# neu-vi/Superpoints_Registration

Measured on AMD Instinct MI355X. Metric: point-cloud pairs/sec (16 384 pts/cloud), higher is better.
Workload: dtype f32 (matrix products: range-scaled split-f16x2 MFMA, f32 accumulate; attention weights below 2^-5 of their row sum carried in one f16 plane); 1 GPU; synthetic 16384-pt pairs, full KPConv backbone + superpoint attn + Sinkhorn-SVD pose (3dmatch config, BASELINE configs[1]); streams_per_gpu=1, points_per_cloud=16384, generator=box, point_order=reference, upsample_indices=True, cross_step_overlap=True, streams_inside_a_forward=3: main path, pyramid searches, ResNet shortcut branches

## Files before the change

superpoints_registration_amd/csrc/norm_pool.hip:

```cpp
#include "spr_common.h"

namespace spr {
namespace {

constexpr int kSliceRows = 512;
int in_nsplit(int max_len) {
  int s = cdiv(max_len > 0 ? max_len : 1, kSliceRows);
  return s < 1 ? 1 : s;
}

__global__ __launch_bounds__(256) void k_in_stats(const float* __restrict__ x,
                                                  const int* __restrict__ cu, int c, int nsplit,
                                                  double* __restrict__ part ) {
  const int cloud = blockIdx.x, split = blockIdx.y, cb = blockIdx.z * 64;
  const int beg = cu[cloud], end = cu[cloud + 1];
  const int r0 = beg + split * kSliceRows;
  const int r1 = min(r0 + kSliceRows, end);
  const int cw = min(c - cb, 64);
  const int cw4 = cw >> 2;
  const int rl = 256 / cw4;
  const int tc = threadIdx.x % cw4, tr = threadIdx.x / cw4;
  __shared__ double sh[8][256];
  double s[4] = {0, 0, 0, 0}, ss[4] = {0, 0, 0, 0};
  if (tr < rl) {
    const float* base = x + cb + 4 * tc;
    int r = r0 + tr;
    for (; r + 3 * rl < r1; r += 4 * rl) {
      float4 v[4];
#pragma unroll
      for (int u = 0; u < 4; ++u)
        v[u] = *reinterpret_cast<const float4*>(base + (size_t)(r + u * rl) * c);
#pragma unroll
      for (int u = 0; u < 4; ++u) {
        const double a = v[u].x, b = v[u].y, cc = v[u].z, d = v[u].w;
        s[0] += a; ss[0] += a * a;
        s[1] += b; ss[1] += b * b;
        s[2] += cc; ss[2] += cc * cc;
        s[3] += d; ss[3] += d * d;
      }
    }
    for (; r < r1; r += rl) {
      const float4 v = *reinterpret_cast<const float4*>(base + (size_t)r * c);
      const double a = v.x, b = v.y, cc = v.z, d = v.w;
      s[0] += a; ss[0] += a * a;
      s[1] += b; ss[1] += b * b;
      s[2] += cc; ss[2] += cc * cc;
      s[3] += d; ss[3] += d * d;
    }
  }
#pragma unroll
  for (int k = 0; k < 4; ++k) {
    sh[k][threadIdx.x] = s[k];
    sh[4 + k][threadIdx.x] = ss[k];
  }
  __syncthreads();
  if (tr == 0) {
    double* p = part + (((size_t)cloud * nsplit + split) * 2) * c;
#pragma unroll
    for (int k = 0; k < 4; ++k) {
      double a = s[k], b = ss[k];
      for (int q = 1; q < rl; ++q) {
        a += sh[k][q * cw4 + tc];
        b += sh[4 + k][q * cw4 + tc];
      }
      p[cb + 4 * tc + k] = a;
      p[c + cb + 4 * tc + k] = b;
    }
  }
}

__global__ void k_in_final(const double* __restrict__ part, const int* __restrict__ cu, int nb,
                           int c, int nsplit, float eps, float* __restrict__ mean,
                           float* __restrict__ rstd) {
  const int i = blockIdx.x * blockDim.x + threadIdx.x;
  if (i >= nb * c) return;
  const int cloud = i / c, ch = i % c;
  double s = 0.0, ss = 0.0;
  for (int k = 0; k < nsplit; ++k) {
    const double* p = part + (((size_t)cloud * nsplit + k) * 2) * c;
    s += p[ch];
    ss += p[c + ch];
  }
  const int len = cu[cloud + 1] - cu[cloud];
  const double n = len > 0 ? (double)len : 1.0;
  const double m = s / n;
  double var = ss / n - m * m;
  if (var < 0.0) var = 0.0;
  mean[i] = (float)m;
  rstd[i] = (float)(1.0 / sqrt(var + (double)eps));
}

__device__ __forceinline__ void publish_range(float mx, float* __restrict__ slots, int nslots) {
  __shared__ float shr[4];
  mx = wave_max(mx);
  if ((threadIdx.x & 63) == 0) shr[threadIdx.x >> 6] = mx;
  __syncthreads();
  if (threadIdx.x == 0)
    atomicMax(reinterpret_cast<unsigned int*>(slots) + (blockIdx.x & (nslots - 1)),
              __float_as_uint(fmaxf(fmaxf(shr[0], shr[1]), fmaxf(shr[2], shr[3]))));
}

constexpr int kInApplyUnroll = 4;
__global__ __launch_bounds__(256) void k_in_apply(const float* __restrict__ x, const int* __restrict__ cu, int n,
                                                  int nb, int c, int norm, const float* __restrict__ mean,
                                                  const float* __restrict__ rstd, const float* __restrict__ add,
                                                  float slope, float* __restrict__ out,
                                                  float* __restrict__ out_range, int nslots) {
  const int c4 = c >> 2;
  const long total = (long)n * c4;
  const long stride = (long)gridDim.x * blockDim.x;
  const long g0 = (long)blockIdx.x * blockDim.x + threadIdx.x;
  float4 v[kInApplyUnroll], a[kInApplyUnroll];
#pragma unroll
  for (int u = 0; u < kInApplyUnroll; ++u) {
    const long gid = g0 + u * stride;
    if (gid < total) {
      v[u] = reinterpret_cast<const float4*>(x)[gid];
      if (add) a[u] = reinterpret_cast<const float4*>(add)[gid];
    }
  }
  float mx = 0.f;
#pragma unroll
  for (int u = 0; u < kInApplyUnroll; ++u) {
    const long gid = g0 + u * stride;
    if (gid >= total) continue;
    float4 w = v[u];
    if (norm) {
      const int row = (int)(gid / c4), q = (int)(gid % c4);
      const int cloud = find_segment(cu, nb, row);
      const float4 m = reinterpret_cast<const float4*>(mean + (size_t)cloud * c)[q];
      const float4 r = reinterpret_cast<const float4*>(rstd + (size_t)cloud * c)[q];
      w.x = (w.x - m.x) * r.x;
      w.y = (w.y - m.y) * r.y;
      w.z = (w.z - m.z) * r.z;
      w.w = (w.w - m.w) * r.w;
    }
    if (add) {
      w.x += a[u].x;
      w.y += a[u].y;
      w.z += a[u].z;
      w.w += a[u].w;
    }
    w.x = w.x >= 0.f ? w.x : w.x * slope;
    w.y = w.y >= 0.f ? w.y : w.y * slope;
    w.z = w.z >= 0.f ? w.z : w.z * slope;
    w.w = w.w >= 0.f ? w.w : w.w * slope;
    reinterpret_cast<float4*>(out)[gid] = w;
    mx = fmaxf(mx, fmaxf(fmaxf(fabsf(w.x), fabsf(w.y)), fmaxf(fabsf(w.z), fabsf(w.w))));
  }
  if (out_range != nullptr) publish_range(mx, out_range, nslots);
}

__global__ __launch_bounds__(256) void k_in_bwd_stats(const float* __restrict__ x, const float* __restrict__ out,
                                                      const float* __restrict__ dout, const int* __restrict__ cu,
                                                      int c, int nsplit, float slope,
                                                      const float* __restrict__ mean, const float* __restrict__ rstd,
                                                      double* __restrict__ part ) {
  const int cloud = blockIdx.x, split = blockIdx.y, cb = blockIdx.z * 64;
  const int beg = cu[cloud], end = cu[cloud + 1];
  const int r0 = beg + split * kSliceRows;
  const int r1 = min(r0 + kSliceRows, end);
  const int cw = min(c - cb, 64);
  const int cw4 = cw >> 2;
  const int rl = 256 / cw4;
  const int tc = threadIdx.x % cw4, tr = threadIdx.x / cw4;
  __shared__ double sh[8][256];
  double s1[4] = {0, 0, 0, 0}, s2[4] = {0, 0, 0, 0};
  if (tr < rl) {
    const int col = cb + 4 * tc;
    const float4 mu = *reinterpret_cast<const float4*>(mean + (size_t)cloud * c + col);
    const float4 rs = *reinterpret_cast<const float4*>(rstd + (size_t)cloud * c + col);
    for (int r = r0 + tr; r < r1; r += rl) {
      const size_t o = (size_t)r * c + col;
      const float4 xv = *reinterpret_cast<const float4*>(x + o);
      const float4 ov = *reinterpret_cast<const float4*>(out + o);
      const float4 dv = *reinterpret_cast<const float4*>(dout + o);
      const float g0 = dv.x * (ov.x > 0.f ? 1.f : slope), g1 = dv.y * (ov.y > 0.f ? 1.f : slope);
      const float g2 = dv.z * (ov.z > 0.f ? 1.f : slope), g3 = dv.w * (ov.w > 0.f ? 1.f : slope);
      s1[0] += (double)g0; s2[0] += (double)g0 * (double)((xv.x - mu.x) * rs.x);
      s1[1] += (double)g1; s2[1] += (double)g1 * (double)((xv.y - mu.y) * rs.y);
      s1[2] += (double)g2; s2[2] += (double)g2 * (double)((xv.z - mu.z) * rs.z);
      s1[3] += (double)g3; s2[3] += (double)g3 * (double)((xv.w - mu.w) * rs.w);
    }
  }
#pragma unroll
  for (int k = 0; k < 4; ++k) {
    sh[k][threadIdx.x] = s1[k];
    sh[4 + k][threadIdx.x] = s2[k];
  }
  __syncthreads();
  if (tr == 0) {
    double* p = part + (((size_t)cloud * nsplit + split) * 2) * c;
#pragma unroll
    for (int k = 0; k < 4; ++k) {
      double a = s1[k], b = s2[k];
      for (int q = 1; q < rl; ++q) {
        a += sh[k][q * cw4 + tc];
        b += sh[4 + k][q * cw4 + tc];
      }
      p[cb + 4 * tc + k] = a;
      p[c + cb + 4 * tc + k] = b;
    }
  }
}

__global__ void k_in_bwd_final(const double* __restrict__ part, const int* __restrict__ cu, int nb, int c,
                               int nsplit, double* __restrict__ m1, double* __restrict__ m2) {
  const int i = blockIdx.x * blockDim.x + threadIdx.x;
  if (i >= nb * c) return;
  const int cloud = i / c, ch = i % c;
  double s1 = 0.0, s2 = 0.0;
  for (int k = 0; k < nsplit; ++k) {
    const double* p = part + (((size_t)cloud * nsplit + k) * 2) * c;
    s1 += p[ch];
    s2 += p[c + ch];
  }
  const int len = cu[cloud + 1] - cu[cloud];
  const double n = len > 0 ? (double)len : 1.0;
  m1[i] = s1 / n;
  m2[i] = s2 / n;
}

__global__ void k_in_bwd_apply(const float* __restrict__ x, const float* __restrict__ out,
                               const float* __restrict__ dout, const int* __restrict__ cu, int n, int nb, int c,
                               int norm, float slope, const float* __restrict__ mean,
                               const float* __restrict__ rstd, const double* __restrict__ m1,
                               const double* __restrict__ m2, float* __restrict__ dx, float* __restrict__ dadd) {
  const long gid = (long)blockIdx.x * blockDim.x + threadIdx.x;
  if (gid >= (long)n * c) return;
  const int row = (int)(gid / c), ch = (int)(gid % c);
  const float g = dout[gid] * (out[gid] > 0.f ? 1.f : slope);
  if (dadd) dadd[gid] = g;
  if (!norm) {
    dx[gid] = g;
    return;
  }
  const int cloud = find_segment(cu, nb, row);
  const size_t s = (size_t)cloud * c + ch;
  const float xh = (x[gid] - mean[s]) * rstd[s];
  dx[gid] = rstd[s] * (float)(((double)g - m1[s]) - (double)xh * m2[s]);
}

__global__ void k_in_bwd_apply4(const float* __restrict__ x, const float* __restrict__ out,
                                const float* __restrict__ dout, const int* __restrict__ cu, int n, int nb, int c,
                                int norm, float slope, const float* __restrict__ mean,
                                const float* __restrict__ rstd, const double* __restrict__ m1,
                                const double* __restrict__ m2, float* __restrict__ dx, float* __restrict__ dadd) {
  const int c4 = c >> 2;
  const long gid = (long)blockIdx.x * blockDim.x + threadIdx.x;
  if (gid >= (long)n * c4) return;
  const int row = (int)(gid / c4), ch = 4 * (int)(gid % c4);
  const float4 d4 = reinterpret_cast<const float4*>(dout)[gid], o4 = reinterpret_cast<const float4*>(out)[gid];
  float g[4] = {d4.x * (o4.x > 0.f ? 1.f : slope), d4.y * (o4.y > 0.f ? 1.f : slope),
                d4.z * (o4.z > 0.f ? 1.f : slope), d4.w * (o4.w > 0.f ? 1.f : slope)};
  if (dadd) reinterpret_cast<float4*>(dadd)[gid] = make_float4(g[0], g[1], g[2], g[3]);
  if (!norm) {
    reinterpret_cast<float4*>(dx)[gid] = make_float4(g[0], g[1], g[2], g[3]);
    return;
  }
  const int cloud = find_segment(cu, nb, row);
  const size_t s = (size_t)cloud * c + ch;
  const float4 x4 = reinterpret_cast<const float4*>(x)[gid];
  const float xv[4] = {x4.x, x4.y, x4.z, x4.w};
  float r[4];
#pragma unroll
  for (int e = 0; e < 4; ++e) {
    const float xh = (xv[e] - mean[s + e]) * rstd[s + e];
    r[e] = rstd[s + e] * (float)(((double)g[e] - m1[s + e]) - (double)xh * m2[s + e]);
  }
  reinterpret_cast<float4*>(dx)[gid] = make_float4(r[0], r[1], r[2], r[3]);
}

__global__ void k_maxpool(const float* __restrict__ x, int ns, int c, const int* __restrict__ idx,
                          int nq, int idx_stride, int k, float* __restrict__ out, float* __restrict__ out_range,
                          int nslots, const int* __restrict__ order) {
  const int c4 = c >> 2;
  long gid = (long)blockIdx.x * blockDim.x + threadIdx.x;
  if (order != nullptr) gid = ((long)(blockIdx.x & 7) * (gridDim.x >> 3) + (blockIdx.x >> 3)) * blockDim.x + threadIdx.x;
  float mx = 0.f;
  if (gid < (long)nq * c4) {
  const int q = (int)(gid % c4);
  const int row = order != nullptr ? order[gid / c4] : (int)(gid / c4);
  gid = (long)row * c4 + q;
  float4 m = make_float4(-INFINITY, -INFINITY, -INFINITY, -INFINITY);
  const int* ir = idx + (size_t)row * idx_stride;
  int j = 0;
  for (; j + 4 <= k; j += 4) {
    int id[4];
    float4 v[4];
#pragma unroll
    for (int u = 0; u < 4; ++u) id[u] = ir[j + u];
#pragma unroll
    for (int u = 0; u < 4; ++u) {
      v[u] = make_float4(0.f, 0.f, 0.f, 0.f);
      if (id[u] >= 0 && id[u] < ns) v[u] = reinterpret_cast<const float4*>(x + (size_t)id[u] * c)[q];
    }
#pragma unroll
    for (int u = 0; u < 4; ++u) {
      m.x = fmaxf(m.x, v[u].x);
      m.y = fmaxf(m.y, v[u].y);
      m.z = fmaxf(m.z, v[u].z);
      m.w = fmaxf(m.w, v[u].w);
    }
  }
  for (; j < k; ++j) {
    const int id = ir[j];
    float4 v = make_float4(0.f, 0.f, 0.f, 0.f);
    if (id >= 0 && id < ns) v = reinterpret_cast<const float4*>(x + (size_t)id * c)[q];
    m.x = fmaxf(m.x, v.x);
    m.y = fmaxf(m.y, v.y);
    m.z = fmaxf(m.z, v.z);
    m.w = fmaxf(m.w, v.w);
  }
  reinterpret_cast<float4*>(out)[gid] = m;
  mx = fmaxf(fmaxf(fabsf(m.x), fabsf(m.y)), fmaxf(fabsf(m.z), fabsf(m.w)));
  }
  if (out_range != nullptr) publish_range(mx, out_range, nslots);
}

__global__ void k_gather_rows(const float* __restrict__ x, int n_src, int c,
                              const int* __restrict__ idx, int n, float* __restrict__ out) {
  const long gid = (long)blockIdx.x * blockDim.x + threadIdx.x;
  if (gid >= (long)n * c) return;
  const int row = (int)(gid / c), ch = (int)(gid % c);
  const int id = idx[row];
  out[gid] = (id >= 0 && id < n_src) ? x[(size_t)id * c + ch] : 0.f;
}

}
}

using namespace spr;

extern "C" size_t spr_instnorm_workspace_bytes(int max_len, int nb, int c) {
  const size_t B = (size_t)(nb > 0 ? nb : 1), C = (size_t)(c > 0 ? c : 1);
  const int ns = in_nsplit(max_len);
  return align_up(B * ns * 2 * C * sizeof(double), 256) + 2 * align_up(B * C * sizeof(float), 256);
}

extern "C" int spr_instnorm(const float* x, const int* cu, int n, int nb, int max_len_host, int c,
                            float eps, int norm, const float* add, float slope, float* out, float* out_range,
                            int out_range_n, void* ws, size_t ws_bytes, void* stream_) {
  hipStream_t stream = (hipStream_t)stream_;
  SPR_REQUIRE(out_range == nullptr || (out_range_n >= 1 && (out_range_n & (out_range_n - 1)) == 0),
              "instnorm: out_range_n must be a power of two");
  SPR_REQUIRE(n > 0 && nb >= 1 && c >= 4 && c % 4 == 0, "instnorm: need n>0 and c %% 4 == 0 (c=%d)", c);
  float* mean = nullptr;
  float* rstd = nullptr;
  if (norm) {
    SPR_REQUIRE(max_len_host >= 1 && max_len_host <= n, "instnorm: bad max_len_host=%d", max_len_host);
    SPR_REQUIRE(ws_bytes >= spr_instnorm_workspace_bytes(max_len_host, nb, c), "instnorm: workspace too small");
    Workspace w(ws, ws_bytes);
    const int nsplit = in_nsplit(max_len_host);
    double* part = w.take<double>((size_t)nb * nsplit * 2 * c);
    mean = w.take<float>((size_t)nb * c);
    rstd = w.take<float>((size_t)nb * c);
    SPR_REQUIRE(rstd != nullptr, "instnorm: workspace carve failed");
    hipLaunchKernelGGL(k_in_stats, dim3(nb, nsplit, cdiv(c, 64)), dim3(256), 0, stream, x, cu, c, nsplit, part);
    hipLaunchKernelGGL(k_in_final, dim3(cdiv((long)nb * c, 256)), dim3(256), 0, stream, part, cu,
                       nb, c, nsplit, eps, mean, rstd);
    SPR_LAUNCH_CHECK();
  }
  const long total = (long)n * (c / 4);
  hipLaunchKernelGGL(k_in_apply, dim3(cdiv(total, 256 * kInApplyUnroll)), dim3(256), 0, stream, x, cu, n, nb, c,
                     norm, mean, rstd, add, slope, out, out_range, out_range_n);
  SPR_LAUNCH_CHECK();
  return 0;
}

extern "C" int spr_instnorm_stats(const float* x, const int* cu, int n, int nb, int max_len_host, int c, float eps,
                                  float* mean, float* rstd, void* ws, size_t ws_bytes, void* stream_) {
  hipStream_t stream = (hipStream_t)stream_;
  SPR_REQUIRE(x && cu && mean && rstd && n > 0 && nb >= 1 && c >= 4 && c % 4 == 0, "instnorm_stats: bad arguments (c=%d)", c);
  SPR_REQUIRE(max_len_host >= 1 && max_len_host <= n, "instnorm_stats: bad max_len_host=%d", max_len_host);
  SPR_REQUIRE(ws_bytes >= spr_instnorm_workspace_bytes(max_len_host, nb, c), "instnorm_stats: workspace too small");
  Workspace w(ws, ws_bytes);
  const int nsplit = in_nsplit(max_len_host);
  double* part = w.take<double>((size_t)nb * nsplit * 2 * c);
  SPR_REQUIRE(part != nullptr, "instnorm_stats: workspace carve failed");
  hipLaunchKernelGGL(k_in_stats, dim3(nb, nsplit, cdiv(c, 64)), dim3(256), 0, stream, x, cu, c, nsplit, part);
  hipLaunchKernelGGL(k_in_final, dim3(cdiv((long)nb * c, 256)), dim3(256), 0, stream, part, cu, nb, c, nsplit, eps, mean,
                     rstd);
  SPR_LAUNCH_CHECK();
  return 0;
}

extern "C" size_t spr_instnorm_bwd_workspace_bytes(int max_len, int nb, int c) {
  const size_t B = (size_t)(nb > 0 ? nb : 1), C = (size_t)(c > 0 ? c : 1);
  return spr_instnorm_workspace_bytes(max_len, nb, c) + 2 * align_up(B * C * sizeof(double), 256);
}

extern "C" int spr_instnorm_bwd(const float* x, const float* out, const float* dout, const int* cu, int n, int nb,
                                int max_len_host, int c, float eps, int norm, float slope, float* dx, float* dadd,
                                void* ws, size_t ws_bytes, void* stream_) {
  hipStream_t stream = (hipStream_t)stream_;
  SPR_REQUIRE(n > 0 && nb >= 1 && c >= 4 && c % 4 == 0, "instnorm_bwd: need n>0 and c %% 4 == 0 (c=%d)", c);
  SPR_REQUIRE(x && out && dout && dx, "instnorm_bwd: null operand");
  float *mean = nullptr, *rstd = nullptr;
  double *m1 = nullptr, *m2 = nullptr;
  if (norm) {
    SPR_REQUIRE(max_len_host >= 1 && max_len_host <= n, "instnorm_bwd: bad max_len_host=%d", max_len_host);
    SPR_REQUIRE(ws_bytes >= spr_instnorm_bwd_workspace_bytes(max_len_host, nb, c), "instnorm_bwd: workspace too small");
    Workspace w(ws, ws_bytes);
    const int nsplit = in_nsplit(max_len_host);
    double* part = w.take<double>((size_t)nb * nsplit * 2 * c);
    mean = w.take<float>((size_t)nb * c);
    rstd = w.take<float>((size_t)nb * c);
    m1 = w.take<double>((size_t)nb * c);
    m2 = w.take<double>((size_t)nb * c);
    SPR_REQUIRE(m2 != nullptr, "instnorm_bwd: workspace carve failed");
    hipLaunchKernelGGL(k_in_stats, dim3(nb, nsplit, cdiv(c, 64)), dim3(256), 0, stream, x, cu, c, nsplit, part);
    hipLaunchKernelGGL(k_in_final, dim3(cdiv((long)nb * c, 256)), dim3(256), 0, stream, part, cu, nb, c, nsplit,
                       eps, mean, rstd);
    hipLaunchKernelGGL(k_in_bwd_stats, dim3(nb, nsplit, cdiv(c, 64)), dim3(256), 0, stream, x, out, dout, cu, c, nsplit, slope,
                       mean, rstd, part);
    hipLaunchKernelGGL(k_in_bwd_final, dim3(cdiv((long)nb * c, 256)), dim3(256), 0, stream, part, cu, nb, c, nsplit,
                       m1, m2);
    SPR_LAUNCH_CHECK();
  }
  if (c % 4 == 0 && (((uintptr_t)x | (uintptr_t)out | (uintptr_t)dout | (uintptr_t)dx | (uintptr_t)dadd) & 15) == 0)
    hipLaunchKernelGGL(k_in_bwd_apply4, dim3(cdiv((long)n * (c / 4), 256)), dim3(256), 0, stream, x, out, dout, cu, n, nb,
                       c, norm, slope, mean, rstd, m1, m2, dx, dadd);
  else
    hipLaunchKernelGGL(k_in_bwd_apply, dim3(cdiv((long)n * c, 256)), dim3(256), 0, stream, x, out, dout, cu, n, nb, c,
                       norm, slope, mean, rstd, m1, m2, dx, dadd);
  SPR_LAUNCH_CHECK();
  return 0;
}

extern "C" int spr_maxpool_gather(const float* x, int ns, int c, const int* idx, int nq, int idx_stride, int k,
                                  const int* order, float* out, float* out_range, int out_range_n, void* stream_) {
  hipStream_t stream = (hipStream_t)stream_;
  SPR_REQUIRE(out_range == nullptr || (out_range_n >= 1 && (out_range_n & (out_range_n - 1)) == 0),
              "maxpool: out_range_n must be a power of two");
  SPR_REQUIRE(nq > 0 && ns > 0 && c % 4 == 0 && k >= 1 && k <= idx_stride, "maxpool: bad arguments");
  const long total = (long)nq * (c / 4);
  const long nblk = order != nullptr ? align_up((size_t)cdiv(total, 256), 8) : cdiv(total, 256);
  hipLaunchKernelGGL(k_maxpool, dim3((unsigned)nblk), dim3(256), 0, stream, x, ns, c, idx, nq, idx_stride, k, out,
                     out_range, out_range_n, order);
  SPR_LAUNCH_CHECK();
  return 0;
}

extern "C" int spr_gather_rows(const float* x, int n_src, int c, const int* idx, int n, float* out,
                               void* stream_) {
  hipStream_t stream = (hipStream_t)stream_;
  SPR_REQUIRE(n > 0 && c >= 1, "gather_rows: bad arguments");
  const long total = (long)n * c;
  hipLaunchKernelGGL(k_gather_rows, dim3(cdiv(total, 256)), dim3(256), 0, stream, x, n_src, c, idx,
                     n, out);
  SPR_LAUNCH_CHECK();
  return 0;
}
```

superpoints_registration_amd/ops.py:

```python
import ctypes
import math
import threading
from typing import Optional, Sequence, Tuple

import numpy as np
import torch

from . import _lib

ACT_NONE, ACT_RELU, ACT_SIGMOID = 0, 1, 2
ORDER_REFERENCE, ORDER_CANONICAL = 0, 1


def _stream(t: torch.Tensor):
    return ctypes.c_void_p(torch.cuda.current_stream(t.device).cuda_stream)


def _ptr(t: Optional[torch.Tensor]):
    return None if t is None else ctypes.c_void_p(t.data_ptr())


def _dev(t: torch.Tensor, name: str, dtype=None) -> torch.Tensor:
    if not isinstance(t, torch.Tensor) or not t.is_cuda:
        raise RuntimeError(f"{name} must be a tensor on the MI355X device (got "
# ... 354 lines not shown
    status = torch.zeros((max(nb, 1),), dtype=torch.int32, device=dev)
    _lib.check(L.spr_augment_pairs(
        _ptr(src_xyz), _ptr(src_cu), ns, _ptr(tgt_xyz), _ptr(tgt_cu), nt, _ptr(pose), nb, _ptr(src_mask), _ptr(tgt_mask),
        _ptr(corr), stride, _ptr(off_d), _ptr(cnt_d), _ptr(perturb_d), _ptr(flags), AUG_MODES[mode], float(scale),
        int(max_pts), int(seed), _ptr(pk_dev), _ptr(noise), _ptr(keys), _ptr(o_src), _ptr(o_tgt), _ptr(o_scu),
        _ptr(o_tcu), _ptr(o_pose), _ptr(o_smask), _ptr(o_tmask), _ptr(o_sperm), _ptr(o_tperm), _ptr(out_corr),
        _ptr(out_cnt), _ptr(status), _ptr(ws), ws.numel(), _stream(src_xyz)), "spr_augment_pairs")
    out = {'src_xyz': o_src, 'tgt_xyz': o_tgt, 'src_cu': o_scu, 'tgt_cu': o_tcu, 'pose': o_pose, 'src_perm': o_sperm,
           'tgt_perm': o_tperm, 'status': status[:nb]}
    if src_mask is not None:
        out['src_mask'], out['tgt_mask'] = o_smask.view(torch.bool), o_tmask.view(torch.bool)
    if corr is not None:
        out['corr'], out['corr_count'] = out_corr, out_cnt
    return out


class RadiusTable:

    def __init__(self, supports: torch.Tensor, s_cu: torch.Tensor, radius: float):
        self.supports = _dev(supports, "supports", torch.float32)
        self.s_cu = _dev(s_cu, "s_cu", torch.int32)
        self.radius = float(radius)
        self.ns, self.nb = self.supports.shape[0], self.s_cu.numel() - 1
        L = _lib.lib()
        self.blob = torch.empty((L.spr_radius_table_bytes(self.ns, self.nb),), dtype=torch.uint8, device=supports.device)
        ws = _workspace(L.spr_radius_table_build_workspace_bytes(self.ns, self.nb), supports.device)
        _lib.check(L.spr_radius_table_build(_ptr(self.supports), _ptr(self.s_cu), self.ns, self.nb, self.radius,
                                            _ptr(self.blob), self.blob.numel(), _ptr(ws), ws.numel(),
                                            _stream(self.supports)), "spr_radius_table_build")
        self._slot = 0
        self._slots = L.spr_radius_table_slots()
        self._versions = (self.supports._version, self.s_cu._version)

    def matches(self, supports: torch.Tensor, s_cu: torch.Tensor, radius: float) -> bool:
        return (supports.data_ptr() == self.supports.data_ptr() and supports.shape[0] == self.ns
                and s_cu.data_ptr() == self.s_cu.data_ptr() and float(radius) == self.radius
                and (self.supports._version, self.s_cu._version) == self._versions
                and supports._version == self.supports._version and s_cu._version == self.s_cu._version
                and self._slot < self._slots)

    def query(self, queries: torch.Tensor, q_cu: torch.Tensor, limit: int,
              dense: Optional[bool] = None) -> Tuple[torch.Tensor, int]:
        queries = _dev(queries, "queries", torch.float32)
        q_cu = _dev(q_cu, "q_cu", torch.int32)
        nq = queries.shape[0]
        self_search = int(queries.data_ptr() == self.supports.data_ptr() and nq == self.ns
                          and q_cu.data_ptr() == self.s_cu.data_ptr())
        L = _lib.lib()
        ws = _workspace(L.spr_radius_table_query_workspace_bytes(nq), queries.device)
        out = torch.empty((nq, limit), dtype=torch.int32, device=queries.device)
        mc = torch.empty((1,), dtype=torch.int32, device=queries.device)
        slot, self._slot = self._slot, self._slot + 1
        _lib.check(L.spr_radius_table_query(_ptr(queries), _ptr(q_cu), nq, self_search, self.ns, self.nb, self.radius,
                                            int(limit), slot, _ptr(self.blob), _ptr(out), _ptr(mc),
                                            -1 if dense is None else int(bool(dense)), _ptr(ws), ws.numel(),
                                            _stream(queries)), "spr_radius_table_query")
        m = int(mc.item())
        if m == -2:
            return radius_neighbors(queries, self.supports, q_cu, self.s_cu, self.radius, limit, True, algo=1)
        if m < 0:
            raise RuntimeError("spr_radius_neighbors: cloud extent / radius exceeds 8191 cells per axis")
        if m < 1:
            raise RuntimeError("Error")
        return out[:, :min(m, limit)], m


def _wants_grad(*tensors) -> bool:
    return torch.is_grad_enabled() and any(isinstance(t, torch.Tensor) and t.requires_grad for t in tensors)


def kpconv(q_pts, s_pts, nbr, x, weights, kernel_points, kp_extent: float, rows_sorted: bool = False,
           impl: int = 0) -> torch.Tensor:
    if _wants_grad(x, weights):
        from .autograd import KPConvFn
        return KPConvFn.apply(_dev(q_pts, "q_pts", torch.float32), _dev(s_pts, "s_pts", torch.float32), nbr,
                              _dev(x, "x", torch.float32), weights, kernel_points, float(kp_extent),
                              bool(rows_sorted), int(impl))
    return kpconv_raw(q_pts, s_pts, nbr, x, weights, kernel_points, kp_extent, rows_sorted, impl)


def kpconv_raw(q_pts, s_pts, nbr, x, weights, kernel_points, kp_extent: float, rows_sorted: bool = False,
               impl: int = 0, order: Optional[torch.Tensor] = None) -> torch.Tensor:
    q_pts = _dev(q_pts, "q_pts", torch.float32)
    s_pts = _dev(s_pts, "s_pts", torch.float32)
    x = _dev(x, "x", torch.float32)
    weights = _dev(weights, "weights", torch.float32)
    kernel_points = _dev(kernel_points, "kernel_points", torch.float32)
    if not nbr.is_cuda:
        raise RuntimeError("neighb_inds must be on the device")
    if nbr.dtype != torch.int32:
        nbr = nbr.to(torch.int32)
    stride = nbr.stride(0) if nbr.stride(1) == 1 and nbr.shape[1] > 0 else None
    if stride is None:
        nbr = nbr.contiguous()
        stride = nbr.shape[1]
    nq, ns, kmax = q_pts.shape[0], s_pts.shape[0], nbr.shape[1]
    n_kp, cin, cout = weights.shape
    assert x.shape == (ns, cin), (x.shape, ns, cin)
    L = _lib.lib()
    ws = _workspace(L.spr_kpconv_workspace_bytes(nq, ns, cin, cout), x.device)
    out = torch.empty((nq, cout), dtype=torch.float32, device=x.device)
    xr, xr_n = _get_range(x)
    wr, wr_n = _static_range(weights)
    plan = wplanes = None
    if impl == 0 and n_kp == 15 and cin % 32 == 0 and cout % 32 == 0 and cout <= 256:
        if cin in (32, 64) and cin * cout <= 4096 and kmax <= 128:
            plan = _kpconv_plan(nbr, nq, ns, int(stride), kmax, bool(rows_sorted), order)
        if wr is not None:
            wplanes = _kpconv_wplanes(weights, wr, wr_n)
    _lib.check(L.spr_kpconv_fwd(_ptr(q_pts), nq, _ptr(s_pts), ns, _ptr(nbr), int(stride), kmax,
                                int(bool(rows_sorted)), _ptr(x), cin, _ptr(weights), cout,
                                _ptr(kernel_points), n_kp, float(kp_extent), _ptr(out), int(impl),
                                _ptr(xr), int(xr_n), _ptr(wr), int(wr_n), _ptr(plan), _ptr(wplanes),
                                _ptr(ws), ws.numel(), _stream(x)), "spr_kpconv_fwd")
    return out


def _kpconv_plan(nbr: torch.Tensor, nq: int, ns: int, stride: int, kmax: int, rows_sorted: bool,
                 order: Optional[torch.Tensor] = None) -> torch.Tensor:
    if order is not None:
        order = _dev(order, "order", torch.int32)
        assert order.shape == (nq,)
    key = (nbr.data_ptr(), nbr._version, nq, ns, stride, kmax, rows_sorted, _range_epoch[0],
           None if order is None else (order.data_ptr(), order._version))
    c = getattr(nbr, '_spr_kp_plan', None)
    if c is not None and c[0] == key:
        c[2].acquire()
        return c[1]
    L = _lib.lib()
    nbytes = L.spr_kpconv_plan_bytes(nq)
    plan = torch.empty((nbytes,), dtype=torch.uint8, device=nbr.device)
    _lib.check(L.spr_kpconv_plan(_ptr(nbr), nq, ns, stride, kmax, int(rows_sorted), _ptr(order), _ptr(plan), nbytes,
                                 _stream(nbr)), "spr_kpconv_plan")
    nbr._spr_kp_plan = (key, plan, _StreamGuard(plan))
    return plan


def kpconv_plan_prefetch(nbr: torch.Tensor, ns: int, rows_sorted: bool = True) -> None:
    if nbr is None or not nbr.is_cuda or nbr.dtype != torch.int32 or nbr.dim() != 2 or nbr.shape[1] < 1:
        return
    if nbr.stride(1) != 1 or nbr.shape[1] > 128 or nbr.shape[0] < 1:
        return
    _kpconv_plan(nbr, nbr.shape[0], int(ns), int(nbr.stride(0)), nbr.shape[1], bool(rows_sorted))


def _kpconv_wplanes(weights: torch.Tensor, wr: torch.Tensor, wr_n: int) -> torch.Tensor:
    key = (weights.data_ptr(), weights._version, wr.data_ptr(), _range_epoch[0])
    c = getattr(weights, '_spr_kp_wplanes', None)
    if c is not None and c[0] == key:
        c[2].acquire()
        return c[1]
    L = _lib.lib()
    n_kp, cin, cout = weights.shape
    nbytes = L.spr_kpconv_wplanes_bytes(cin, cout)
    planes = torch.empty((nbytes,), dtype=torch.uint8, device=weights.device)
    _lib.check(L.spr_kpconv_prep_weights(_ptr(weights), n_kp, cin, cout, _ptr(wr), int(wr_n), _ptr(planes), nbytes,
                                         _stream(weights)), "spr_kpconv_prep_weights")
    weights._spr_kp_wplanes = (key, planes, _StreamGuard(planes))
    return planes


def instnorm(x, cu, eps: float = 1e-5, norm: bool = True, add=None, slope: float = 1.0,
             out=None, max_len: Optional[int] = None) -> torch.Tensor:
    if _wants_grad(x, add):
        from .autograd import InstNormFn
        return InstNormFn.apply(_dev(x, "x", torch.float32), _dev(cu, "cu", torch.int32), float(eps), bool(norm),
                                None if add is None else _dev(add, "add", torch.float32), float(slope), max_len)
    return instnorm_raw(x, cu, eps, norm, add, slope, out, max_len)


def instnorm_raw(x, cu, eps: float = 1e-5, norm: bool = True, add=None, slope: float = 1.0,
                 out=None, max_len: Optional[int] = None) -> torch.Tensor:
    x = _dev(x, "x", torch.float32)
    cu = _dev(cu, "cu", torch.int32)
    n, c = x.shape
    nb = cu.numel() - 1
    if add is not None:
        add = _dev(add, "add", torch.float32)
        assert add.shape == x.shape
    if out is None:
        out = torch.empty_like(x)
    L = _lib.lib()
    max_len = n if max_len is None else max(1, min(int(max_len), n))
    ws = _workspace(L.spr_instnorm_workspace_bytes(max_len, nb, c), x.device)
    cnt = _STREAM_SLOTS
    rng = _zero_slots(cnt, x.device)
    _lib.check(L.spr_instnorm(_ptr(x), _ptr(cu), n, nb, max_len, c, float(eps), int(bool(norm)), _ptr(add),
                              float(slope), _ptr(out), _ptr(rng), cnt, _ptr(ws), ws.numel(), _stream(x)),
               "spr_instnorm")
    _set_range(out, rng, cnt)
    return out


def block_tail_tile_rows(ka: int, kb: int, n_out: int) -> int:
    if _modes["gemm"] != 1:
        return 0
    return int(_lib.lib().spr_block_tail_tile_rows(int(ka), int(kb), int(n_out)))


def _tail_tiles(cu: torch.Tensor, n: int, tr: int) -> torch.Tensor:
    key = (cu.data_ptr(), cu._version, n, tr, _range_epoch[0])
    cache = getattr(cu, '_spr_tail_tiles', None)
    if cache is None:
        cache = {}
        cu._spr_tail_tiles = cache
    c = cache.get(tr)
    if c is not None and c[0] == key:
        c[2].acquire()
        return c[1]
    L = _lib.lib()
    t = torch.empty((L.spr_block_tail_tiles_len(n, cu.numel() - 1, tr),), dtype=torch.int32, device=cu.device)
    _lib.check(L.spr_block_tail_tiles(_ptr(cu), n, cu.numel() - 1, tr, _ptr(t), _stream(cu)), "spr_block_tail_tiles")
    cache[tr] = (key, t, _StreamGuard(t))
    return t


def instnorm_stats(x, cu, eps: float = 1e-5, max_len: Optional[int] = None):
    x = _dev(x, "x", torch.float32)
    cu = _dev(cu, "cu", torch.int32)
    n, c = x.shape
    nb = cu.numel() - 1
    L = _lib.lib()
    max_len = n if max_len is None else max(1, min(int(max_len), n))
    ws = _workspace(L.spr_instnorm_workspace_bytes(max_len, nb, c), x.device)
    st = torch.empty((2, nb, c), dtype=torch.float32, device=x.device)
    _lib.check(L.spr_instnorm_stats(_ptr(x), _ptr(cu), n, nb, max_len, c, float(eps), _ptr(st[0]), _ptr(st[1]),
                                    _ptr(ws), ws.numel(), _stream(x)), "spr_instnorm_stats")
    return st[0], st[1]


_NORM_BOUNDS = {}


def _norm_bound(max_len: int, device) -> torch.Tensor:
    key = (int(max_len), str(device))
    t = _NORM_BOUNDS.get(key)
    if t is None:
        t = torch.full((1,), float(max(1, int(max_len))) ** 0.5, dtype=torch.float32, device=device)
        _NORM_BOUNDS[key] = t
    return t


def block_tail(xa, wa, cu, xb=None, wb=None, add=None, eps: float = 1e-5, slope: float = 0.1,
               xa_stats=None, xa_slope: float = 0.1, xa_max_len: Optional[int] = None) -> torch.Tensor:
    xa = _dev(xa, "xa", torch.float32)
    wa = _dev(wa, "wa", torch.float32)
    cu = _dev(cu, "cu", torch.int32)
    n, ka = xa.shape
    n_out = wa.shape[0]
    assert wa.shape[1] == ka
    kb = 0
    if xb is not None:
        xb = _dev(xb, "xb", torch.float32)
        wb = _dev(wb, "wb", torch.float32)
        kb = xb.shape[1]
        assert xb.shape[0] == n and wb.shape == (n_out, kb) and add is None
    if add is not None:
        add = _dev(add, "add", torch.float32)
        assert add.shape == (n, n_out)
    nb = cu.numel() - 1
    L = _lib.lib()
    tr = L.spr_block_tail_tile_rows(ka, kb, n_out)
    if tr <= 0:
        raise RuntimeError(f"block_tail: no kernel for ka={ka} kb={kb} n_out={n_out}")
    tiles = _tail_tiles(cu, n, tr)
    out = torch.empty((n, n_out), dtype=torch.float32, device=xa.device)
    ws = _workspace(L.spr_block_tail_workspace_bytes(n, nb, kb, n_out, tr), xa.device)
    if xa_stats is not None:
        xar, xar_n = _norm_bound(n if xa_max_len is None else xa_max_len, xa.device), 1
    else:
        xar, xar_n = _get_range(xa)
    war, war_n = _static_range(wa)
    xbr, xbr_n, wbr, wbr_n = None, 0, None, 0
    if kb > 0:
        xbr, xbr_n = _get_range(xb)
        wbr, wbr_n = _static_range(wb)
    cnt = _STREAM_SLOTS
    rng = _zero_slots(cnt, xa.device)
    mean = rstd = None
    if xa_stats is not None:
        mean, rstd = xa_stats
        assert mean.shape == (nb, ka) and rstd.shape == (nb, ka) and mean.is_contiguous() and rstd.is_contiguous()
    _lib.check(L.spr_block_tail(_ptr(xa), ka, _ptr(wa), _ptr(xb), kb, _ptr(wb), _ptr(add), _ptr(cu), _ptr(tiles),
                                n, nb, n_out, float(eps), float(slope), _ptr(out), _ptr(xar), int(xar_n),
                                _ptr(war), int(war_n), _ptr(xbr), int(xbr_n), _ptr(wbr), int(wbr_n),
                                _ptr(rng), cnt, _ptr(mean), _ptr(rstd), float(xa_slope), _ptr(ws), ws.numel(),
                                _stream(xa)), "spr_block_tail")
    _set_range(out, rng, cnt)
    return out


def cell_order(points: torch.Tensor, cu: torch.Tensor, cell: float) -> torch.Tensor:
    points = _dev(points, "points", torch.float32)
    cu = _dev(cu, "cu", torch.int32)
    n, nb = points.shape[0], cu.numel() - 1
    L = _lib.lib()
    out = torch.empty((n,), dtype=torch.int32, device=points.device)
    ws = _workspace(L.spr_cell_order_workspace_bytes(n), points.device)
    _lib.check(L.spr_cell_order(_ptr(points), _ptr(cu), n, nb, float(cell), _ptr(out), _ptr(ws), ws.numel(),
                                _stream(points)), "spr_cell_order")
    return out


def maxpool(x, idx, order=None) -> torch.Tensor:
    if _wants_grad(x):
        from .autograd import MaxPoolFn
        return MaxPoolFn.apply(_dev(x, "x", torch.float32), idx)
    return maxpool_raw(x, idx, order)


def maxpool_raw(x, idx, order=None) -> torch.Tensor:
    x = _dev(x, "x", torch.float32)
    if idx.dtype != torch.int32:
        idx = idx.to(torch.int32)
    stride = idx.stride(0) if idx.stride(1) == 1 else None
    if stride is None:
        idx = idx.contiguous()
        stride = idx.shape[1]
    ns, c = x.shape
    nq, k = idx.shape
    out = torch.empty((nq, c), dtype=torch.float32, device=x.device)
    L = _lib.lib()
    cnt = _STREAM_SLOTS
    rng = _zero_slots(cnt, x.device)
    if order is not None and (order.dtype != torch.int32 or order.numel() != nq or not order.is_contiguous()):
        raise ValueError("maxpool: order must be a contiguous int32 permutation of the query rows")
    _lib.check(L.spr_maxpool_gather(_ptr(x), ns, c, _ptr(idx), nq, int(stride), k, _ptr(order), _ptr(out),
                                    _ptr(rng), cnt, _stream(x)), "spr_maxpool_gather")
    _set_range(out, rng, cnt)
    return out


def linear(x, weight, bias=None, residual=None, act: int = ACT_NONE) -> torch.Tensor:
    if _wants_grad(x, weight, bias, residual):
        from .autograd import LinearFn
        return LinearFn.apply(_dev(x, "x", torch.float32), weight, bias, residual, int(act))
    return linear_raw(x, weight, bias, residual, act)


def linear_raw(x, weight, bias=None, residual=None, act: int = ACT_NONE) -> torch.Tensor:
    x = _dev(x, "x", torch.float32)
    weight = _dev(weight, "weight", torch.float32)
    m, k = x.shape
    n = weight.shape[0]
    assert weight.shape[1] == k
    if bias is not None:
        bias = _dev(bias, "bias", torch.float32)
    if residual is not None:
        residual = _dev(residual, "residual", torch.float32)
        assert residual.shape == (m, n)
    out = torch.empty((m, n), dtype=torch.float32, device=x.device)
    L = _lib.lib()
    ws = _workspace(L.spr_linear_workspace_bytes(), x.device)
    xr, xr_n = _get_range(x)
    wr, wr_n = _static_range(weight)
    orng = torch.empty((_RANGE_CAP,), dtype=torch.float32, device=x.device) if residual is None else None
    on = ctypes.c_int(0)
    _lib.check(L.spr_linear(_ptr(x), m, k, _ptr(weight), n, _ptr(bias), _ptr(residual), int(act), _ptr(out),
                            _ptr(xr), int(xr_n), _ptr(wr), int(wr_n), _ptr(orng),
                            _RANGE_CAP if orng is not None else 0, ctypes.byref(on),
                            _ptr(ws), ws.numel(), _stream(x)), "spr_linear")
    if orng is not None:
        _set_range(out, orng, on.value)
    return out


DEFAULT_ATTN_MODE = 4

_modes = {"gemm": 1, "attn": DEFAULT_ATTN_MODE}


def set_gemm_mode(mode: int) -> None:
    _lib.check(_lib.lib().spr_set_gemm_mode(int(mode)), "spr_set_gemm_mode")
    _modes["gemm"] = int(mode)


def layernorm(x, gamma, beta, eps: float = 1e-5, pos=None, want_norm: bool = True):
    if _wants_grad(x, gamma, beta):
        from .autograd import LayerNormFn
        n, p = LayerNormFn.apply(_dev(x, "x", torch.float32), gamma, beta, float(eps), pos, bool(want_norm))
        return (n if (want_norm or pos is None) else None), (p if pos is not None else None)
    return layernorm_raw(x, gamma, beta, eps, pos, want_norm)


def layernorm_raw(x, gamma, beta, eps: float = 1e-5, pos=None, want_norm: bool = True):
    x = _dev(x, "x", torch.float32)
    m, c = x.shape
    out_norm = torch.empty_like(x) if want_norm else None
    out_pos = None
    if pos is not None:
        pos = _dev(pos, "pos", torch.float32)
        out_pos = torch.empty_like(x)
    L = _lib.lib()
    cnt = L.spr_layernorm_range_count(m)
    rn = _zero_slots(cnt, x.device) if out_norm is not None else None
    rp = _zero_slots(cnt, x.device) if out_pos is not None else None
    _lib.check(L.spr_layernorm(_ptr(x), m, c, _ptr(_dev(gamma, "gamma", torch.float32)),
                               _ptr(_dev(beta, "beta", torch.float32)), float(eps), _ptr(pos),
                               _ptr(out_norm), _ptr(out_pos), _ptr(rn), _ptr(rp), _stream(x)), "spr_layernorm")
    if out_norm is not None:
        _set_range(out_norm, rn, cnt)
    if out_pos is not None:
        _set_range(out_pos, rp, cnt)
    return out_norm, out_pos


def posemb_sine(xyz, d_model: int, scale: float = 1.0, temperature: float = 10000.0) -> torch.Tensor:
    xyz = _dev(xyz, "xyz", torch.float32)
    n = xyz.shape[0]
    out = torch.empty((n, d_model), dtype=torch.float32, device=xyz.device)
    _lib.check(_lib.lib().spr_posemb_sine(_ptr(xyz), n, d_model, float(scale * 2 * math.pi),
                                          float(temperature), _ptr(out), _stream(xyz)),
               "spr_posemb_sine")
    return out


def attention(q, k, v, cu, kv_seg, max_len: int, nhead: int, out=None, lens_host=None,
              kv_seg_host=None) -> torch.Tensor:
    if _wants_grad(q, k, v):
        from .autograd import AttentionFn
        if lens_host is None:
            c = cu.cpu().tolist()
            lens_host = [c[i + 1] - c[i] for i in range(len(c) - 1)]
        if kv_seg_host is None:
            kv_seg_host = kv_seg.cpu().tolist()
        return AttentionFn.apply(q, k, v, _dev(cu, "cu", torch.int32), _dev(kv_seg, "kv_seg", torch.int32),
                                 int(max_len), int(nhead), list(lens_host), list(kv_seg_host))
    return attention_raw(q, k, v, cu, kv_seg, max_len, nhead, out)


def attention_raw(q, k, v, cu, kv_seg, max_len: int, nhead: int, out=None, want_lse: bool = False):
    for t, nm in ((q, "q"), (k, "k"), (v, "v")):
        if not t.is_cuda or t.dtype != torch.float32 or t.stride(1) != 1:
            raise RuntimeError(f"attention: {nm} must be a float32 device tensor with unit inner stride")
    T, d = q.shape
    hd = d // nhead
    cu = _dev(cu, "cu", torch.int32)
    kv_seg = _dev(kv_seg, "kv_seg", torch.int32)
    nseg = cu.numel() - 1
    if out is None:
        out = torch.empty((T, d), dtype=torch.float32, device=q.device)
    L = _lib.lib()
    ws = _workspace(L.spr_attn_workspace_bytes(T, nseg, nhead, hd), q.device)
    lse = torch.empty((T, nhead), dtype=torch.float32, device=q.device) if want_lse else None
    written = ctypes.c_int(0)
    _lib.check(L.spr_attn_varlen_fwd(_ptr(q), q.stride(0), _ptr(k), k.stride(0), _ptr(v), v.stride(0),
                                     _ptr(cu), _ptr(kv_seg), T, nseg, int(max_len), nhead, hd,
                                     1.0 / math.sqrt(hd), _ptr(out), out.stride(0), _ptr(lse),
                                     ctypes.byref(written), _ptr(ws), ws.numel(), _stream(q)),
               "spr_attn_varlen_fwd")
    if want_lse:
        return out, (lse if written.value else None)
    return out


def attention_probs(q, k, cu, kv_seg, max_len: int, nhead: int, average: bool = True, out=None, place=None,
                    max_rows: Optional[int] = None, max_cols: Optional[int] = None) -> torch.Tensor:
    for t, nm in ((q, "q"), (k, "k")):
        if not isinstance(t, torch.Tensor) or not t.is_cuda:
            raise RuntimeError(f"attention_probs: {nm} must be a tensor on the MI355X device; the HIP path has no "
                               "CPU fallback")
        if t.dtype != torch.float32 or t.stride(1) != 1:
            raise RuntimeError(f"attention_probs: {nm} must be float32 with unit inner stride")
    q, k = q.detach(), k.detach()
    T, d = q.shape
    hd = d // nhead
    cu = _dev(cu, "cu", torch.int32)
    kv_seg = _dev(kv_seg, "kv_seg", torch.int32)
    nseg = cu.numel() - 1
    L = int(max_len)
    if out is None:
        if place is not None:
            raise RuntimeError("attention_probs: `place` needs `out`")
        shape = (nseg, L, L) if average else (nseg, nhead, L, L)
        out = torch.empty(shape, dtype=torch.float32, device=q.device)
        per = L * L * (1 if average else nhead)
        pl = np.zeros((nseg, 5), dtype=np.int64)
        pl[:, 0] = np.arange(nseg, dtype=np.int64) * per
        pl[:, 1], pl[:, 2], pl[:, 3], pl[:, 4] = L, L * L, L, L
        place, max_rows, max_cols = pl, L, L
    else:
        if not out.is_cuda or out.dtype != torch.float32 or not out.is_contiguous():
            raise RuntimeError("attention_probs: out must be a contiguous float32 device tensor")
        if place is None:
            raise RuntimeError("attention_probs: `out` needs `place`")
    if isinstance(place, np.ndarray) or (isinstance(place, torch.Tensor) and not place.is_cuda):
        pl = np.asarray(place.cpu().numpy() if isinstance(place, torch.Tensor) else place, dtype=np.int64)
        if pl.shape != (nseg, 5):
            raise RuntimeError(f"attention_probs: place must be [nseg={nseg}, 5] (got {pl.shape})")
        nh = 1 if average else nhead
        last = pl[:, 0] + (nh - 1) * pl[:, 2] + (pl[:, 3] - 1) * pl[:, 1] + pl[:, 4]
        if (pl[:, 0] < 0).any() or (pl[:, 3] < 1).any() or (pl[:, 4] < 1).any() or (pl[:, 4] > pl[:, 1]).any() \
                or int(last.max()) > out.numel():
            raise RuntimeError("attention_probs: place describes entries outside `out`")
        max_rows, max_cols = int(pl[:, 3].max()), int(pl[:, 4].max())
        place = torch.from_numpy(pl).to(q.device)
    elif max_rows is None or max_cols is None:
        raise RuntimeError("attention_probs: a device `place` needs max_rows and max_cols")
    Lb = _lib.lib()
    ws = _workspace(Lb.spr_attn_probs_workspace_bytes(T, nhead, hd), q.device)
    _lib.check(Lb.spr_attn_probs(_ptr(q), q.stride(0), _ptr(k), k.stride(0), _ptr(cu), _ptr(kv_seg), T, nseg, L,
                                 nhead, hd, 1.0 / math.sqrt(hd), 0 if average else 1, _ptr(out), _ptr(place),
                                 int(max_rows), int(max_cols), _ptr(ws), ws.numel(), _stream(q)), "spr_attn_probs")
    return out


_seg_perm_cache = {}


def _segment_perms(kv_seg_host, device):
    key = (tuple(int(x) for x in kv_seg_host), str(device))
    c = _seg_perm_cache.get(key)
    if c is None:
        kv = np.asarray(key[0], dtype=np.int32)
        inv = np.empty_like(kv)
        inv[kv] = np.arange(kv.size, dtype=np.int32)
        c = (torch.from_numpy(kv).to(device), torch.from_numpy(inv).to(device))
        _seg_perm_cache[key] = c
    return c


def attention_bwd(q, k, v, out, dout, cu, kv_seg_host, max_len: int, nhead: int, lse=None):
    for t, nm in ((q, "q"), (k, "k"), (v, "v"), (out, "out"), (dout, "dout")):
        if not t.is_cuda or t.dtype != torch.float32 or t.stride(1) != 1:
            raise RuntimeError(f"attention_bwd: {nm} must be a float32 device tensor with unit inner stride")
    T, d = q.shape
    hd = d // nhead
    cu = _dev(cu, "cu", torch.int32)
    nseg = cu.numel() - 1
    kv, inv = _segment_perms(kv_seg_host, q.device)
    dq = torch.empty((T, d), dtype=torch.float32, device=q.device)
    dk = torch.empty_like(dq)
    dv = torch.empty_like(dq)
    L = _lib.lib()
    ws = _workspace(L.spr_attn_bwd_workspace_bytes(T, nseg, nhead), q.device)
    _lib.check(L.spr_attn_varlen_bwd(_ptr(q), q.stride(0), _ptr(k), k.stride(0), _ptr(v), v.stride(0), _ptr(out),
                                     out.stride(0), _ptr(dout), dout.stride(0), _ptr(lse), _ptr(cu), _ptr(kv),
                                     _ptr(inv), T, nseg, int(max_len), nhead, hd, 1.0 / math.sqrt(hd), _ptr(dq),
                                     _ptr(dk), _ptr(dv), _ptr(ws), ws.numel(), _stream(q)), "spr_attn_varlen_bwd")
    return dq, dk, dv


def inproj_prepare(w_in: torch.Tensor):
    r = getattr(w_in, '_spr_inproj', None)
    if r is not None and r[1] == w_in._version and r[2] == w_in.data_ptr() and r[3] == _range_epoch[0]:
        r[4].acquire()
        return r[0]
    L = _lib.lib()
    d = w_in.shape[1]
    buf = torch.empty((L.spr_range_parts() + 3 * d,), dtype=torch.float32, device=w_in.device)
    _lib.check(L.spr_attn_inproj_prepare(_ptr(w_in), d, _ptr(buf), _stream(w_in)), "spr_attn_inproj_prepare")
    w_in._spr_inproj = (buf, w_in._version, w_in.data_ptr(), _range_epoch[0], _StreamGuard(buf))
    return buf


def attention_inproj(x_qk, x_v, w_in, b_in, cu, kv_seg, max_len: int, nhead: int, w_prep=None) -> torch.Tensor:
    x_qk = _dev(x_qk, "x_qk", torch.float32)
    x_v = x_qk if x_v is x_qk else _dev(x_v, "x_v", torch.float32)
    w_in = _dev(w_in, "w_in", torch.float32)
    b_in = _dev(b_in, "b_in", torch.float32)
    T, d = x_qk.shape
    assert x_v.shape == (T, d) and w_in.shape == (3 * d, d) and b_in.shape == (3 * d,)
    hd = d // nhead
    cu = _dev(cu, "cu", torch.int32)
    kv_seg = _dev(kv_seg, "kv_seg", torch.int32)
    nseg = cu.numel() - 1
    out = torch.empty((T, d), dtype=torch.float32, device=x_qk.device)
    L = _lib.lib()
    ws = _workspace(L.spr_attn_inproj_workspace_bytes(T, nseg, nhead, hd), x_qk.device)
    fused = _modes["attn"] != 0 and _modes["gemm"] == 1 and T >= 256
    qr, qn = _get_range(x_qk) if fused else (None, 0)
    vr, vn = (qr, qn) if x_v is x_qk else (_get_range(x_v) if fused else (None, 0))
    orng = torch.empty((1,), dtype=torch.float32, device=x_qk.device) if fused else None
    _lib.check(L.spr_attn_inproj_varlen_fwd(_ptr(x_qk), _ptr(x_v), T, _ptr(w_in), _ptr(b_in), _ptr(cu),
                                            _ptr(kv_seg), nseg, int(max_len), nhead, hd, 1.0 / math.sqrt(hd),
                                            _ptr(out), out.stride(0), _ptr(qr), int(qn), _ptr(vr), int(vn),
                                            _ptr(orng), _ptr(w_prep if fused else None), _ptr(ws), ws.numel(),
                                            _stream(x_qk)),
               "spr_attn_inproj_varlen_fwd")
    if orng is not None:
        _set_range(out, orng, 1)
    return out


_xenc_lock = threading.Lock()
XENC_PTRS_PER_LAYER = 18


class XencPlan:

    def __init__(self, key, prepared, plan, keep):
        self.key, self.prepared, self.plan, self.keep = key, prepared, plan, keep

    def __deepcopy__(self, memo):
        return None

    def __reduce__(self):
        return (_no_plan, ())


def _no_plan():
    return None


def xenc_available() -> bool:
    return _modes["gemm"] == 1 and _modes["attn"] in (1, 2, 3, 4)
# ... 354 lines not shown
```

Baseline: 1234 pairs/s.

## Add LDS-tiled max-pool that deduplicates neighbour rows per query tile

Adds a max-pool kernel for the ordered path. Each block takes 32 spatially ordered queries and deduplicates their neighbour indices with an LDS hash table. It then stages the unique source rows into LDS in 32-channel slabs and computes each query's max from LDS. The goal is to cut repeated global gathers of the same neighbour rows across nearby queries. The cost is hashing, a prefix scan and extra barriers, plus a fallback path when more than 448 unique rows are needed.

Result: slower. 1208 pairs/s (-2.1%).

```diff
diff --git a/superpoints_registration_amd/csrc/norm_pool.hip b/superpoints_registration_amd/csrc/norm_pool.hip
--- a/superpoints_registration_amd/csrc/norm_pool.hip
+++ b/superpoints_registration_amd/csrc/norm_pool.hip
@@ -318,6 +318,190 @@
   if (out_range != nullptr) publish_range(mx, out_range, nslots);
 }
 
+constexpr int kMpTQ = 32;
+constexpr int kMpCH = 32;
+constexpr int kMpCap = 448;
+constexpr int kMpG = kMpCH / 4;
+constexpr int kMpQPP = 256 / kMpG;
+constexpr int kMpStage = 8;
+static_assert(256 % kMpG == 0 && kMpTQ % kMpQPP == 0 && kMpTQ <= 256, "max-pool tile shape");
+
+__host__ __device__ constexpr size_t mp_tile_lds(int ks, int ht) {
+  return (size_t)(kMpCap + 1) * kMpCH * 4 + ((size_t)ht + (size_t)kMpTQ * ks + kMpCap + kMpTQ + 8) * 4;
+}
+
+__global__ __launch_bounds__(256) void k_maxpool_tile(const float* __restrict__ x, int ns, int c,
+                                                      const int* __restrict__ idx, int nq, int idx_stride, int k,
+                                                      float* __restrict__ out, float* __restrict__ out_range,
+                                                      int nslots, const int* __restrict__ order, int ht_log2) {
+  extern __shared__ __align__(16) unsigned char mp_lds[];
+  const int tid = threadIdx.x;
+  const int ht = 1 << ht_log2, ks = (k + 3) & ~3, c4 = c >> 2;
+  float4* rows = reinterpret_cast<float4*>(mp_lds);
+  int* tab = reinterpret_cast<int*>(rows + (kMpCap + 1) * kMpG);
+  int* sidx = tab + ht;
+  int* rowid = sidx + kMpTQ * ks;
+  int* srow = rowid + kMpCap;
+  int* scan = srow + kMpTQ;
+  const long q0 = ((long)(blockIdx.x & 7) * (gridDim.x >> 3) + (blockIdx.x >> 3)) * kMpTQ;
+  const int nqt = q0 < nq ? (int)min((long)kMpTQ, nq - q0) : 0;
+  float mx = 0.f;
+  if (nqt > 0) {
+    for (int i = tid; i < ht; i += 256) tab[i] = -1;
+    if (tid < kMpG) rows[kMpCap * kMpG + tid] = make_float4(0.f, 0.f, 0.f, 0.f);
+    if (tid < nqt) srow[tid] = order[q0 + tid];
+    const int nent = nqt * ks;
+    for (int e = tid; e < nent; e += 256) {
+      const int ql = e / ks, j = e - ql * ks;
+      int id = -1;
+      if (j < k) {
+        id = idx[(size_t)order[q0 + ql] * idx_stride + j];
+        if (id >= ns) id = -1;
+      }
+      sidx[e] = id < 0 ? -1 : id;
+    }
+    __syncthreads();
+    for (int e = tid; e < nent; e += 256) {
+      const int id = sidx[e];
+      if (id < 0) continue;
+      unsigned int h = ((unsigned int)id * 2654435761u) >> (32 - ht_log2);
+      int cell = -1;
+      for (int p = 0; p < ht; ++p) {
+        const int prev = atomicCAS(&tab[h], -1, id);
+        if (prev == -1 || prev == id) {
+          cell = (int)h;
+          break;
+        }
+        h = (h + 1) & (unsigned int)(ht - 1);
+      }
+      sidx[e] = cell;
+    }
+    __syncthreads();
+    int mine = 0;
+    for (int i = tid; i < ht; i += 256) mine += tab[i] >= 0 ? 1 : 0;
+    int incl = mine;
+#pragma unroll
+    for (int o = 1; o < 64; o <<= 1) {
+      const int t = __shfl_up(incl, o, 64);
+      if ((tid & 63) >= o) incl += t;
+    }
+    if ((tid & 63) == 63) scan[tid >> 6] = incl;
+    __syncthreads();
+    int base = incl - mine;
+    for (int w = 0; w < (tid >> 6); ++w) base += scan[w];
+    const int nrows = scan[0] + scan[1] + scan[2] + scan[3];
+    if (nrows <= kMpCap) {
+      for (int i = tid; i < ht; i += 256) {
+        const int id = tab[i];
+        if (id >= 0) {
+          rowid[base] = id;
+          tab[i] = base++;
+        }
+      }
+      __syncthreads();
+      for (int e = tid; e < nent; e += 256) {
+        const int cell = sidx[e];
+        sidx[e] = cell >= 0 ? tab[cell] : kMpCap;
+      }
+      __syncthreads();
+      const int g = tid % kMpG, qlane = tid / kMpG;
+      const int npiece = nrows * kMpG;
+      for (int cb = 0; cb < c4; cb += kMpG) {
+        const int gw = min(kMpG, c4 - cb);
+        if (g < gw) {
+          for (int p0 = tid; p0 < npiece; p0 += 256 * kMpStage) {
+            float4 v[kMpStage];
+#pragma unroll
+            for (int u = 0; u < kMpStage; ++u) {
+              const int p = min(p0 + u * 256, npiece - kMpG + g);
+              v[u] = reinterpret_cast<const float4*>(x)[(size_t)rowid[p / kMpG] * c4 + cb + g];
+            }
+#pragma unroll
+            for (int u = 0; u < kMpStage; ++u) {
+              const int p = p0 + u * 256;
+              if (p < npiece) rows[p] = v[u];
+            }
+          }
+        }
+        __syncthreads();
+#pragma unroll 1
+        for (int ql = qlane; ql < nqt; ql += kMpQPP) {
+          if (g >= gw) break;
+          float4 m = make_float4(-INFINITY, -INFINITY, -INFINITY, -INFINITY);
+          const int* sr = sidx + ql * ks;
+          int j = 0;
+          for (; j + 4 <= k; j += 4) {
+            const int4 s = *reinterpret_cast<const int4*>(sr + j);
+            float4 v[4];
+            v[0] = rows[s.x * kMpG + g];
+            v[1] = rows[s.y * kMpG + g];
+            v[2] = rows[s.z * kMpG + g];
+            v[3] = rows[s.w * kMpG + g];
+#pragma unroll
+            for (int u = 0; u < 4; ++u) {
+              m.x = fmaxf(m.x, v[u].x);
+              m.y = fmaxf(m.y, v[u].y);
+              m.z = fmaxf(m.z, v[u].z);
+              m.w = fmaxf(m.w, v[u].w);
+            }
+          }
+          for (; j < k; ++j) {
+            const float4 v = rows[sr[j] * kMpG + g];
+            m.x = fmaxf(m.x, v.x);
+            m.y = fmaxf(m.y, v.y);
+            m.z = fmaxf(m.z, v.z);
+            m.w = fmaxf(m.w, v.w);
+          }
+          reinterpret_cast<float4*>(out)[(size_t)srow[ql] * c4 + cb + g] = m;
+          mx = fmaxf(mx, fmaxf(fmaxf(fabsf(m.x), fabsf(m.y)), fmaxf(fabsf(m.z), fabsf(m.w))));
+        }
+        __syncthreads();
+      }
+    } else {
+      for (int e = tid; e < nent; e += 256) {
+        const int cell = sidx[e];
+        sidx[e] = cell >= 0 ? tab[cell] : -1;
+      }
+      __syncthreads();
+      for (int i = tid; i < nqt * c4; i += 256) {
+        const int ql = i / c4, q = i - ql * c4;
+        float4 m = make_float4(-INFINITY, -INFINITY, -INFINITY, -INFINITY);
+        const int* sr = sidx + ql * ks;
+        int j = 0;
+        for (; j + 4 <= k; j += 4) {
+          const int4 s = *reinterpret_cast<const int4*>(sr + j);
+          const int id[4] = {s.x, s.y, s.z, s.w};
+          float4 v[4];
+#pragma unroll
+          for (int u = 0; u < 4; ++u) {
+            v[u] = make_float4(0.f, 0.f, 0.f, 0.f);
+            if (id[u] >= 0) v[u] = reinterpret_cast<const float4*>(x + (size_t)id[u] * c)[q];
+          }
+#pragma unroll
+          for (int u = 0; u < 4; ++u) {
+            m.x = fmaxf(m.x, v[u].x);
+            m.y = fmaxf(m.y, v[u].y);
+            m.z = fmaxf(m.z, v[u].z);
+            m.w = fmaxf(m.w, v[u].w);
+          }
+        }
+        for (; j < k; ++j) {
+          const int id = sr[j];
+          float4 v = make_float4(0.f, 0.f, 0.f, 0.f);
+          if (id >= 0) v = reinterpret_cast<const float4*>(x + (size_t)id * c)[q];
+          m.x = fmaxf(m.x, v.x);
+          m.y = fmaxf(m.y, v.y);
+          m.z = fmaxf(m.z, v.z);
+          m.w = fmaxf(m.w, v.w);
+        }
+        reinterpret_cast<float4*>(out)[(size_t)srow[ql] * c4 + q] = m;
+        mx = fmaxf(mx, fmaxf(fmaxf(fabsf(m.x), fabsf(m.y)), fmaxf(fabsf(m.z), fabsf(m.w))));
+      }
+    }
+  }
+  if (out_range != nullptr) publish_range(mx, out_range, nslots);
+}
+
 __global__ void k_gather_rows(const float* __restrict__ x, int n_src, int c,
                               const int* __restrict__ idx, int n, float* __restrict__ out) {
   const long gid = (long)blockIdx.x * blockDim.x + threadIdx.x;
@@ -434,6 +618,20 @@
   SPR_REQUIRE(out_range == nullptr || (out_range_n >= 1 && (out_range_n & (out_range_n - 1)) == 0),
               "maxpool: out_range_n must be a power of two");
   SPR_REQUIRE(nq > 0 && ns > 0 && c % 4 == 0 && k >= 1 && k <= idx_stride, "maxpool: bad arguments");
+  if (order != nullptr) {
+    const int ks = (k + 3) & ~3;
+    int ht_log2 = 4;
+    while (ht_log2 < 24 && (1L << ht_log2) < 2L * kMpTQ * ks) ++ht_log2;
+    const size_t lds = mp_tile_lds(ks, 1 << ht_log2);
+    if (ht_log2 < 24 && lds <= 160 * 1024) {
+      if (int rc = ensure_dyn_lds((const void*)k_maxpool_tile, (int)lds)) return rc;
+      const long ntile = (long)align_up((size_t)cdiv(nq, kMpTQ), 8);
+      hipLaunchKernelGGL(k_maxpool_tile, dim3((unsigned)ntile), dim3(256), lds, stream, x, ns, c, idx, nq, idx_stride, k,
+                         out, out_range, out_range_n, order, ht_log2);
+      SPR_LAUNCH_CHECK();
+      return 0;
+    }
+  }
   const long total = (long)nq * (c / 4);
   const long nblk = order != nullptr ? align_up((size_t)cdiv(total, 256), 8) : cdiv(total, 256);
   hipLaunchKernelGGL(k_maxpool, dim3((unsigned)nblk), dim3(256), 0, stream, x, ns, c, idx, nq, idx_stride, k, out,
diff --git a/superpoints_registration_amd/ops.py b/superpoints_registration_amd/ops.py
--- a/superpoints_registration_amd/ops.py
+++ b/superpoints_registration_amd/ops.py
@@ -680,6 +680,9 @@
     return out
 
 
+MAXPOOL_TILE_QUERIES, MAXPOOL_TILE_CHANNELS, MAXPOOL_TILE_ROWS = 32, 32, 448
+
+
 def maxpool(x, idx, order=None) -> torch.Tensor:
     if _wants_grad(x):
         from .autograd import MaxPoolFn
```
